# cloneofsimo/paint-with-words-sd

Hardware: NVIDIA H100
Metric: unet_steps_per_sec_512sq_cfg (higher is better)
Workload: dtype f16

## Files before the change

### paint_with_words_sd_b200/attention.py

```python
from __future__ import annotations

import math
from typing import Dict, Optional, Union

import torch
import torch.nn.functional as F

from . import _native
from .conditioning import PACK_TOKENS, expand_orig_weight_map, key_chunks, pack_weight_map, packed_key, weight_key
from .weight_function import g_of_sigma, probe_weight_function

_ORIG_KEY = "CROSS_ATTENTION_WEIGHT_ORIG"
RECORD_KEY = "ATTN_RECORD"


class _DeviceState:

    def __init__(self, device: torch.device):
        self.device = device
        self.g_sigma = torch.zeros(1, dtype=torch.float32, device=device)
        self._g_key = None
        self.stats = torch.zeros(1024, dtype=torch.float32, device=device)
        self.workspace = torch.zeros(8 << 20, dtype=torch.uint8, device=device)
        self.fused_ws = torch.zeros(_native.lib().pww_xattn_fused_workspace_bytes(), dtype=torch.uint8, device=device)
        self.index_cache: Dict[int, torch.Tensor] = {}
        self.pack_cache: Dict[tuple, object] = {}

    def set_g(self, key, value: float) -> None:
        if key != self._g_key:
            self.g_sigma.fill_(value)
            self._g_key = key

    def ensure(self, batch: int, ws_bytes: int) -> None:
        if self.stats.numel() < batch or self.workspace.numel() < ws_bytes:
            raise _native.NativeError(f"batch of {batch} images exceeds the shim's fixed scratch; split the call or pass "
                                      "your own stats_out/workspace")

    def packed(self, wmap: torch.Tensor):
        key = (wmap.data_ptr(), wmap._version, tuple(wmap.shape), tuple(wmap.stride()))
        hit = self.pack_cache.get(key)
        if hit is None:
            if torch.cuda.is_current_stream_capturing():
                raise _native.NativeError("weight map must be packed before CUDA-graph capture (run one eager step first "
                                          "or pass packed maps)")
            while len(self.pack_cache) >= 16:
                self.pack_cache.pop(next(iter(self.pack_cache)))
            hit = (wmap, pack_weight_map(wmap) or False)
            self.pack_cache[key] = hit
        return hit[1] or None

    def shared_index(self, batch: int) -> torch.Tensor:
        t = self.index_cache.get(batch)
        if t is None:
            t = torch.zeros(batch, dtype=torch.int32, device=self.device)
            self.index_cache[batch] = t
        return t


_STATES: Dict[torch.device, _DeviceState] = {}


def _state(device: torch.device) -> _DeviceState:
    s = _STATES.get(device)
    if s is None:
        s = _STATES[device] = _DeviceState(device)
    return s


def reset_device_state() -> None:
    _STATES.clear()


def resolve_weight_map(context: dict, n: int, device):
    try:
        return context[weight_key(n)]
    except KeyError:
        w = context[_ORIG_KEY]
        if isinstance(w, int):
            if context.get("ORIG_FALLBACK_DROPPED"):
                raise NotImplementedError(
                    f"no CROSS_ATTENTION_WEIGHT_{n} in a multi-image context: the ORIG-map fallback (paint_with_words.py:97-103) "
                    "is a single-image path; use sizes divisible by 64 or one image per sampler")
            return 0
        w = expand_orig_weight_map(w.detach().to("cpu", torch.float32), n).to(device)
        context[weight_key(n)] = w
        return w


def _elem_dtype(q: torch.Tensor) -> torch.dtype:
    return torch.bfloat16 if q.dtype == torch.bfloat16 else torch.float16


def _autocast_dtype(module) -> torch.dtype:
    return torch.bfloat16 if module.to_q.weight.dtype == torch.bfloat16 else torch.float16


def _rows(t: torch.Tensor, dtype: torch.dtype = torch.float16) -> torch.Tensor:
    if t.dtype != dtype:
        t = t.to(dtype)
    if t.stride(-1) != 1 or (t.stride(0) % 8) or (t.stride(1) % 8) or (t.data_ptr() % 16):
        t = t.contiguous()
    return t


XATTN_IMPL = "auto"


def cross_attention(q: torch.Tensor, k: torch.Tensor, v: torch.Tensor, heads: int, scale: float,
                    wmap: Optional[torch.Tensor] = None, wmap_index: Optional[torch.Tensor] = None,
                    stat: Union[int, torch.Tensor] = _native.PWW_STAT_MAX, g_sigma: Optional[torch.Tensor] = None,
                    return_stats: bool = False, packed=None, stats_out: Optional[torch.Tensor] = None,
                    workspace: Optional[torch.Tensor] = None, record=None):
    L = _native.lib()
    dt = _elem_dtype(q)
    q, k, v = _rows(q, dt), _rows(k, dt), _rows(v, dt)
    B, N, C = q.shape
    T = k.shape[1]
    D = C // heads
    if k.stride() != v.stride():
        v = v.contiguous()
        k = k.contiguous()
    st = _state(q.device)
    with torch.cuda.device(q.device):
        out = torch.empty((B, N, C), dtype=dt, device=q.device)
        stream = torch.cuda.current_stream(q.device).cuda_stream
        biased = wmap is not None or packed is not None
        if wmap is not None:
            if wmap.dim() == 2:
                wmap = wmap.unsqueeze(0)
            if wmap.shape[1] != N or wmap.shape[2] != T:
                raise ValueError(f"weight map shape {tuple(wmap.shape)} does not match N={N}, T={T}")
        impl = "dense" if XATTN_IMPL == "dense" else "fused"
        if impl == "dense" and biased and wmap is None:
            impl = "fused"
        if biased and packed is None and impl == "fused":
            if wmap.dtype != torch.float32 or not wmap.is_contiguous():
                wmap = wmap.to(torch.float32).contiguous()
            packed = st.packed(wmap)
        use_fused = impl == "fused" and (not biased or packed is not None)
        if biased and wmap_index is None:
            bw = packed[0].shape[0] if packed is not None else wmap.shape[0]
            wmap_index = st.shared_index(B) if bw == 1 else torch.arange(B, dtype=torch.int32, device=q.device)
        per_image = isinstance(stat, torch.Tensor)
        kind_ptr = None
        if per_image and biased:
            if (stat.dtype != torch.int32 or stat.numel() != B or not stat.is_contiguous() or stat.device != q.device
                    or g_sigma is None or g_sigma.dtype != torch.float32 or g_sigma.numel() != B
                    or not g_sigma.is_contiguous() or g_sigma.device != q.device):
                raise ValueError(f"per-image settings need an int32 [{B}] kind tensor and an fp32 [{B}] G tensor on "
                                 f"{q.device}")
            kind_ptr = stat.data_ptr()
        stats = None
        rec_args = ()
        if record is not None:
            if not use_fused:
                why = ("XATTN_IMPL is 'dense'" if impl == "dense" else
                       "the weight map has more than 10 distinct columns and takes the dense two-launch path")
                raise _native.NativeError(f"attention recording needs the one-launch kernel, but {why}")
            ridx, rec_index, rec_acc = record
            if (ridx.dtype != torch.int8 or ridx.dim() != 2 or ridx.shape[1] != PACK_TOKENS * max(1, key_chunks(T))
                    or not ridx.is_contiguous() or rec_index.dtype != torch.int32 or rec_index.numel() != B
                    or not rec_index.is_contiguous() or rec_acc.dtype != torch.float32 or rec_acc.dim() != 4
                    or tuple(rec_acc.shape[1:]) != (heads, N, 16) or not rec_acc[0].is_contiguous()
                    or any(t.device != q.device for t in (ridx, rec_index, rec_acc))):
                raise ValueError(f"record needs int8 [Br, {PACK_TOKENS * max(1, key_chunks(T))}] ridx, int32 [{B}] "
                                 f"rec_index and fp32 [Br, {heads}, {N}, 16] rec_acc on {q.device}")
            if not per_image and biased:
                stat = torch.full((B,), int(stat), dtype=torch.int32, device=q.device)
                g_sigma = g_sigma.reshape(-1)[:1].expand(B).contiguous()
                kind_ptr, per_image = stat.data_ptr(), True
            rec_args = (ridx.data_ptr(), rec_index.data_ptr(), rec_acc.data_ptr(), rec_acc.stride(0))
        if use_fused:
            mp_ptr = ci_ptr = idx_ptr = g_ptr = st_ptr = ws_ptr = None
            mp_bs = bw = ws_bytes = 0
            if biased:
                mpack, cidx = packed
                if (mpack.shape[1] != N or mpack.dtype != torch.float16 or cidx.dtype != torch.int8
                        or cidx.shape[-1] != PACK_TOKENS * max(1, key_chunks(T))):
                    raise ValueError("packed weight map does not match this attention level")
                st.ensure(B, 0)
                stats = st.stats if stats_out is None else stats_out
                ws = st.fused_ws if workspace is None else workspace
                mp_ptr, ci_ptr, idx_ptr = mpack.data_ptr(), cidx.data_ptr(), wmap_index.data_ptr()
                g_ptr, st_ptr, ws_ptr = g_sigma.data_ptr(), stats.data_ptr(), ws.data_ptr()
                mp_bs, bw, ws_bytes = mpack.stride(0), mpack.shape[0], ws.numel()
            name = "pww_xattn_fused_rec" if rec_args else ("pww_xattn_fused_multi" if per_image else "pww_xattn_fused")
            fn = _native.entry(name, dt)
            rc = fn(q.data_ptr(), k.data_ptr(), v.data_ptr(), out.data_ptr(), B, heads, N, T, D,
                    q.stride(0), q.stride(1), k.stride(0), k.stride(1), out.stride(0), out.stride(1),
                    mp_ptr, mp_bs, bw, ci_ptr, idx_ptr, kind_ptr if per_image or rec_args else stat, g_ptr,
                    float(scale), st_ptr, ws_ptr, ws_bytes, stream, *rec_args)
            _native.check(rc, fn.__name__)
            _native.launch_count += 1
        else:
            stats_ptr = g_ptr = w_ptr = idx_ptr = None
            w_bs = 0
            if biased:
                if wmap is None:
                    raise ValueError("the dense path needs the dense weight map")
                if wmap.dtype != torch.float32 or not wmap.is_contiguous():
                    wmap = wmap.to(torch.float32).contiguous()
                ws_bytes = L.pww_xattn_workspace_bytes(B, heads, N, T, D)
                st.ensure(B, ws_bytes)
                stats = st.stats if stats_out is None else stats_out
                fn = _native.entry("pww_xattn_stats_multi" if per_image else "pww_xattn_stats", dt)
                rc = fn(q.data_ptr(), k.data_ptr(), B, heads, N, T, D, q.stride(0), q.stride(1), k.stride(0),
                        k.stride(1), kind_ptr if per_image else stat, wmap_index.data_ptr(), stats.data_ptr(),
                        st.workspace.data_ptr(), st.workspace.numel(), stream)
                _native.check(rc, fn.__name__)
                _native.launch_count += 1
                stats_ptr, g_ptr = stats.data_ptr(), g_sigma.data_ptr()
                w_ptr, idx_ptr, w_bs = wmap.data_ptr(), wmap_index.data_ptr(), wmap.stride(0)
            fn = _native.entry("pww_xattn_fwd_multi" if per_image else "pww_xattn_fwd", dt)
            rc = fn(q.data_ptr(), k.data_ptr(), v.data_ptr(), out.data_ptr(), B, heads, N, T, D,
                    q.stride(0), q.stride(1), k.stride(0), k.stride(1), out.stride(0), out.stride(1),
                    w_ptr, w_bs, idx_ptr, stats_ptr, g_ptr, float(scale), stream)
            _native.check(rc, fn.__name__)
            _native.launch_count += 1
    if return_stats:
        return out, (stats[:B].clone() if stats is not None else None)
    return out


SELF_ATTN_IMPL = "auto"
SELF_ATTN_NATIVE_MAX_KEYS = 1024


def self_attention(q: torch.Tensor, k: torch.Tensor, v: torch.Tensor, heads: int, scale: float) -> torch.Tensor:
    B, N, C = q.shape
    D = C // heads
    if SELF_ATTN_IMPL == "native" or (SELF_ATTN_IMPL == "auto" and N <= SELF_ATTN_NATIVE_MAX_KEYS):
        dt = _elem_dtype(q)
        fn = _native.entry("pww_attn_fwd", dt)
        q, k, v = _rows(q, dt), _rows(k, dt), _rows(v, dt)
        if not (q.stride() == k.stride() == v.stride()):
            q, k, v = q.contiguous(), k.contiguous(), v.contiguous()
        with torch.cuda.device(q.device):
            out = torch.empty((B, N, C), dtype=dt, device=q.device)
            rc = fn(q.data_ptr(), k.data_ptr(), v.data_ptr(), out.data_ptr(), B, heads, N, D,
                    q.stride(0), q.stride(1), out.stride(0), out.stride(1), float(scale),
                    torch.cuda.current_stream(q.device).cuda_stream)
        _native.check(rc, fn.__name__)
        _native.launch_count += 1
        return out
    qh = q.reshape(B, N, heads, D).transpose(1, 2)
    kh = k.reshape(B, k.shape[1], heads, D).transpose(1, 2)
    vh = v.reshape(B, v.shape[1], heads, D).transpose(1, 2)
    o = F.scaled_dot_product_attention(qh, kh, vh, scale=scale)
    return o.transpose(1, 2).reshape(B, N, C)


def _fused_weight(module, attr: str, names) -> torch.Tensor:
    params = [getattr(module, n).weight for n in names]
    key = tuple((p.data_ptr(), p._version, p.dtype, p.device) for p in params)
    hit = getattr(module, attr, None)
    if hit is None or hit[0] != key:
        hit = (key, torch.cat(params, 0).detach().contiguous())
        object.__setattr__(module, attr, hit)
    return hit[1]


def refresh_kv_cache(context: dict) -> None:
    cache = context.get("KV_CACHE")
    if not cache:
        return
    ctx = context["CONTEXT_TENSOR"]
    for module, kv in cache.values():
        with torch.autocast("cuda", dtype=_autocast_dtype(module)):
            kv.copy_(F.linear(ctx, _fused_weight(module, "_pww_wkv", ("to_k", "to_v"))))


def inj_forward(self, hidden_states, context=None, mask=None):
    if not hidden_states.is_cuda:
        raise _native.NativeError("paint_with_words_sd_b200 attention runs on an H100 GPU only (no CPU path)")
    is_dict = isinstance(context, dict)
    if context is None:
        ctx = hidden_states
    else:
        ctx = context["CONTEXT_TENSOR"] if is_dict else context

    C = self.to_q.weight.shape[0]
    act = _autocast_dtype(self)
    with torch.autocast("cuda", dtype=act):
        if context is None:
            qkv = F.linear(hidden_states, _fused_weight(self, "_pww_wqkv", ("to_q", "to_k", "to_v")))
            q, k, v = qkv[..., :C], qkv[..., C:2 * C], qkv[..., 2 * C:]
        else:
            q = self.to_q(hidden_states)
            cache = context.get("KV_CACHE") if is_dict else None
            hit = cache.get(id(self)) if cache is not None else None
            if hit is not None:
                kv = hit[1]
            else:
                kv = F.linear(ctx, _fused_weight(self, "_pww_wkv", ("to_k", "to_v")))
                if cache is not None:
                    cache[id(self)] = (self, kv)
            k, v = kv[..., :C], kv[..., C:]

    if context is None:
        o = self_attention(q, k, v, self.heads, self.scale)
    else:
        wmap = wmap_index = g_dev = packed = None
        scratch = (None, None)
        stat = _native.PWW_STAT_MAX
        kinds = context.get("STAT_KIND") if is_dict else None
        if kinds is not None:
            w = resolve_weight_map(context, q.shape[1], q.device)
            if isinstance(w, torch.Tensor):
                wmap, stat, g_dev = w, kinds, context["G_SIGMA"]
                wmap_index = context.get("WMAP_INDEX")
                packed = context.get(packed_key(q.shape[1]))
                scratch = context.get("PWW_SCRATCH", scratch)
        elif is_dict:
            f = context["WEIGHT_FUNCTION"]
            sigma = context["SIGMA"]
            w = resolve_weight_map(context, q.shape[1], q.device)
            probed = probe_weight_function(f, sigma)
            if isinstance(w, torch.Tensor) and not probed.is_zero:
                g_dev = context.get("G_SIGMA")
                if g_dev is None:
                    st = _state(q.device)
                    st.set_g((id(f), float(sigma)), g_of_sigma(f, probed, sigma))
                    g_dev = st.g_sigma
                wmap, stat = w, probed.stat
                wmap_index = context.get("WMAP_INDEX")
                packed = context.get(packed_key(q.shape[1]))
                scratch = context.get("PWW_SCRATCH", scratch)
        record = None
        recs = context.get(RECORD_KEY) if is_dict else None
        if recs is not None:
            record = recs.get(q.shape[1])
            if record is None:
                raise _native.NativeError(f"attention recording has no accumulator for N = {q.shape[1]} query rows "
                                          f"(levels: {sorted(recs)})")
        if k.shape[0] != q.shape[0]:
            k = k.expand(q.shape[0], -1, -1)
            v = v.expand(q.shape[0], -1, -1)
        o = cross_attention(q, k, v, self.heads, self.scale, wmap, wmap_index, stat, g_dev, packed=packed,
                            stats_out=scratch[0], workspace=scratch[1], record=record)

    with torch.autocast("cuda", dtype=act):
        o = self.to_out[0](o)
        o = self.to_out[1](o)
    return o


class PwWAttnProcessor:

    def __call__(self, attn, hidden_states, encoder_hidden_states=None, attention_mask=None, **kwargs):
        return inj_forward(attn, hidden_states, encoder_hidden_states, attention_mask)


_PATCHED: Dict[type, object] = {}


def patch_unet(unet, forward=inj_forward) -> int:
    count = 0
    for m in unet.modules():
        if m.__class__.__name__ == "CrossAttention":
            cls = m.__class__
            if cls not in _PATCHED:
                _PATCHED[cls] = cls.__dict__.get("__call__")
            cls.__call__ = forward
            count += 1
    return count


def unpatch_all() -> None:
    for cls, orig in _PATCHED.items():
        if orig is None:
            if "__call__" in cls.__dict__:
                delattr(cls, "__call__")
        else:
            cls.__call__ = orig
    _PATCHED.clear()
```

### paint_with_words_sd_b200/csrc/attn_tc.cuh

```cuda
#pragma once
#include "mma_sm90.cuh"
#include "pww_common.cuh"
#include "xattn_core.cuh"

namespace pww {
namespace fa {

constexpr int kThreads = core::kThreads;
constexpr int kBM = core::kBM;
constexpr int kBN = 64;

template <int D>
struct Cfg {
  using T_ = core::Tile<D>;
  static constexpr uint32_t KVBYTES = kBN * T_::LD * 2;
  static constexpr uint32_t OFF_KV = T_::QBYTES;
  static constexpr uint32_t SMEM = T_::QBYTES + 2 * 2 * KVBYTES;
  static_assert(SMEM <= 232448, "shared memory budget");
};

template <typename E>
struct Params {
  const E* q;
  const E* k;
  const E* v;
  E* out;
  int B, H, N;
  int64_t bs, rs;
  int64_t o_bs, o_rs;
  float scale;
};

template <int D, typename E>
constexpr int kMinBlocks = (D == 80 && std::is_same_v<E, __nv_bfloat16>) ? 1 : 0;

template <int D, typename E>
__global__ void __launch_bounds__(kThreads, kMinBlocks<D, E>) attn_fwd_kernel(const Params<E> p) {
  using C = core::Tile<D>;
  using CF = Cfg<D>;
  extern __shared__ __align__(128) unsigned char smem[];
  const uint32_t smem0 = ptx::smem_u32(smem);
  const int warp = threadIdx.x >> 5, lane = threadIdx.x & 31;
  const int qtiles = (p.N + kBM - 1) / kBM;
  const int bh = blockIdx.x / qtiles, qt = blockIdx.x - bh * qtiles;
  const int b = bh / p.H, h = bh - b * p.H;
  const int row_base = qt * kBM;
  const E* qb = p.q + (int64_t)b * p.bs + h * D;
  const E* kb = p.k + (int64_t)b * p.bs + h * D;
  const E* vb = p.v + (int64_t)b * p.bs + h * D;
  const int ntiles = (p.N + kBN - 1) / kBN;
  auto issue_kv = [&](int j) {
    const uint32_t st = smem0 + CF::OFF_KV + (j & 1) * 2 * CF::KVBYTES;
    const int rows = p.N - j * kBN < kBN ? p.N - j * kBN : kBN;
    core::load_rows<D>(st, kb + (int64_t)j * kBN * p.rs, p.rs, kBN, rows);
    core::load_rows<D>(st + CF::KVBYTES, vb + (int64_t)j * kBN * p.rs, p.rs, kBN, rows);
    ptx::cp_async_commit();
  };
  {
    const int rows = p.N - row_base < kBM ? p.N - row_base : kBM;
    core::load_rows<D>(smem0, qb + (int64_t)row_base * p.rs, p.rs, kBM, rows);
  }
  issue_kv(0);
  uint32_t qa[C::KS][4];
  float o[C::NT][4], m0, m1, l0, l1;
  core::warp_online_begin<D>(o, m0, m1, l0, l1);
  const float sl2 = p.scale * 1.4426950408889634f;
  const uint32_t qs = smem0 + (uint32_t)(warp * 16 * C::LD) * 2u;
#pragma unroll 1
  for (int jt = 0; jt < ntiles; ++jt) {
    if (jt + 1 < ntiles) {
      issue_kv(jt + 1);
      ptx::cp_async_wait<1>();
    } else {
      ptx::cp_async_wait<0>();
    }
    __syncthreads();
    if (jt == 0) {
#pragma unroll
      for (int kk = 0; kk < C::KS; ++kk)
        ptx::ldsm_x4(qs + (uint32_t)((lane & 15) * C::LD + kk * 16 + (lane >> 4) * 8) * 2u, qa[kk][0], qa[kk][1], qa[kk][2], qa[kk][3]);
    }
    const uint32_t ks = smem0 + CF::OFF_KV + (jt & 1) * 2 * CF::KVBYTES, vs = ks + CF::KVBYTES;
    float s[kBN / 8][4];
#pragma unroll
    for (int j = 0; j < kBN / 8; ++j) s[j][0] = s[j][1] = s[j][2] = s[j][3] = 0.f;
#pragma unroll
    for (int kk = 0; kk < C::KS; ++kk) {
#pragma unroll
      for (int jp = 0; jp < kBN / 16; ++jp) {
        const int t = 16 * jp + (lane & 7) + ((lane >> 4) << 3), d = kk * 16 + ((lane >> 3) & 1) * 8;
        uint32_t b0, b1, b2, b3;
        ptx::ldsm_x4(ks + (uint32_t)(t * C::LD + d) * 2u, b0, b1, b2, b3);
        ptx::mma16816<E>(s[2 * jp], qa[kk], b0, b1);
        ptx::mma16816<E>(s[2 * jp + 1], qa[kk], b2, b3);
      }
    }
    core::warp_online_chunk<D, E>(s, p.N - jt * kBN, sl2, vs, lane, o, m0, m1, l0, l1);
    __syncthreads();
  }
  core::warp_online_end<D>(o, l0, l1);
  core::warp_store<D>(o, smem + warp * 16 * C::LD * 2, lane, p.out + (int64_t)b * p.o_bs + h * D, p.o_rs,
                      row_base + warp * 16, p.N);
}

template <int D, typename E>
cudaError_t launch(const void* q, const void* k, const void* v, void* out, int B, int H, int N, int64_t bs, int64_t rs,
                   int64_t o_bs, int64_t o_rs, float scale, cudaStream_t s) {
  using CF = Cfg<D>;
  Params<E> p;
  p.q = (const E*)q; p.k = (const E*)k; p.v = (const E*)v; p.out = (E*)out;
  p.B = B; p.H = H; p.N = N; p.bs = bs; p.rs = rs; p.o_bs = o_bs; p.o_rs = o_rs; p.scale = scale;
  const cudaError_t e = allow_dynamic_smem<attn_fwd_kernel<D, E>>(CF::SMEM);
  if (e != cudaSuccess) return e;
  const long long grid = (long long)B * H * ((N + kBM - 1) / kBM);
  if (grid > 0x7fffffffLL) return cudaErrorInvalidConfiguration;
  attn_fwd_kernel<D, E><<<(unsigned)grid, kThreads, CF::SMEM, s>>>(p);
  return cudaGetLastError();
}

}
}
```

Before: 160.2.

## Split keys across warps, add multistage KV pipeline and ones-column row sums

Rewrites the native self-attention kernel. For short sequences (N<=256) the warps are split into two groups over key blocks and their partial results are merged through shared memory. It adds a 3-stage cp.async pipeline where it fits, and computes the softmax denominator by padding V with a ones column, so the row sum falls out of the PV MMA. It also lowers the native self-attention threshold from 1024 to 256 keys, so the 512px levels with 1024 and 4096 tokens now take the fallback (likely SDPA) path. That trades a small extra MMA column and a combine step for more parallelism on small N.

```diff
diff --git a/paint_with_words_sd_b200/attention.py b/paint_with_words_sd_b200/attention.py
--- a/paint_with_words_sd_b200/attention.py
+++ b/paint_with_words_sd_b200/attention.py
@@ -223,7 +223,7 @@
 
 
 SELF_ATTN_IMPL = "auto"
-SELF_ATTN_NATIVE_MAX_KEYS = 1024
+SELF_ATTN_NATIVE_MAX_KEYS = 256
 
 
 def self_attention(q: torch.Tensor, k: torch.Tensor, v: torch.Tensor, heads: int, scale: float) -> torch.Tensor:
diff --git a/paint_with_words_sd_b200/csrc/attn_tc.cuh b/paint_with_words_sd_b200/csrc/attn_tc.cuh
--- a/paint_with_words_sd_b200/csrc/attn_tc.cuh
+++ b/paint_with_words_sd_b200/csrc/attn_tc.cuh
@@ -7,16 +7,26 @@
 namespace fa {
 
 constexpr int kThreads = core::kThreads;
-constexpr int kBM = core::kBM;
-constexpr int kBN = 64;
-
-template <int D>
+constexpr int kWarps = core::kWarps;
+constexpr uint32_t kSmemMax = 232448;
+
+template <int D, int S, int BN>
 struct Cfg {
+  static_assert(S == 1 || S == 2, "key splits");
+  static_assert(BN % 16 == 0, "P V takes 16 keys per k-step");
   using T_ = core::Tile<D>;
-  static constexpr uint32_t KVBYTES = kBN * T_::LD * 2;
-  static constexpr uint32_t OFF_KV = T_::QBYTES;
-  static constexpr uint32_t SMEM = T_::QBYTES + 2 * 2 * KVBYTES;
-  static_assert(SMEM <= 232448, "shared memory budget");
+  static constexpr int R = kWarps / S;
+  static constexpr int BM = 16 * R;
+  static constexpr int KB = S * BN;
+  static constexpr int NV = T_::NT + 1;
+  static constexpr uint32_t QBYTES = BM * T_::LD * 2;
+  static constexpr uint32_t KVBYTES = KB * T_::LD * 2;
+  static constexpr uint32_t OFF_KV = QBYTES;
+  static constexpr int STAGES = QBYTES + 3 * 2 * KVBYTES <= kSmemMax ? 3 : 2;
+  static constexpr uint32_t SMEM = QBYTES + STAGES * 2 * KVBYTES;
+  static constexpr int PART = NV * 4 + 2;
+  static_assert(SMEM <= kSmemMax, "shared memory budget");
+  static_assert(S == 1 || (uint32_t)(kWarps - R) * 32 * PART * 4 <= STAGES * 2 * KVBYTES, "combine buffer");
 };
 
 template <typename E>
@@ -34,89 +44,227 @@
 template <int D, typename E>
 constexpr int kMinBlocks = (D == 80 && std::is_same_v<E, __nv_bfloat16>) ? 1 : 0;
 
-template <int D, typename E>
+template <int D, int NROWS, typename E>
+__device__ __forceinline__ void load_kv(uint32_t dst, const E* src, int64_t rs, int valid) {
+  using C = core::Tile<D>;
+  constexpr int DCH = D / 8, PIECES = NROWS * DCH;
+#pragma unroll
+  for (int i = 0; i < (PIECES + kThreads - 1) / kThreads; ++i) {
+    const int idx = threadIdx.x + i * kThreads;
+    if (PIECES % kThreads != 0 && idx >= PIECES) break;
+    const int r = idx / DCH, c = idx - r * DCH;
+    const bool ok = r < valid;
+    ptx::cp_async16(dst + (uint32_t)(r * C::LD + c * 8) * 2u, ok ? (const void*)(src + (int64_t)r * rs + c * 8) : (const void*)src,
+                    ok ? 16u : 0u);
+  }
+}
+
+template <int D, typename E, int BN, int NV>
+__device__ __forceinline__ void warp_tile(const uint32_t (&qa)[core::Tile<D>::KS][4], uint32_t ks, uint32_t vs, int kv,
+                                          float sl2, int lane, float (&o)[NV][4], float& m0, float& m1) {
+  using C = core::Tile<D>;
+  constexpr int NJ = BN / 8;
+  float s[NJ][4];
+#pragma unroll
+  for (int j = 0; j < NJ; ++j) s[j][0] = s[j][1] = s[j][2] = s[j][3] = 0.f;
+#pragma unroll
+  for (int kk = 0; kk < C::KS; ++kk) {
+#pragma unroll
+    for (int jp = 0; jp < NJ / 2; ++jp) {
+      const int t = 16 * jp + (lane & 7) + ((lane >> 4) << 3), d = kk * 16 + ((lane >> 3) & 1) * 8;
+      uint32_t b0, b1, b2, b3;
+      ptx::ldsm_x4(ks + (uint32_t)(t * C::LD + d) * 2u, b0, b1, b2, b3);
+      ptx::mma16816<E>(s[2 * jp], qa[kk], b0, b1);
+      ptx::mma16816<E>(s[2 * jp + 1], qa[kk], b2, b3);
+    }
+  }
+  if (kv < BN) {
+#pragma unroll
+    for (int j = 0; j < NJ; ++j)
+#pragma unroll
+      for (int e = 0; e < 4; ++e)
+        if (core::tok(j, e, lane) >= kv) s[j][e] = -INFINITY;
+  }
+  float t0 = -INFINITY, t1 = -INFINITY;
+#pragma unroll
+  for (int j = 0; j < NJ; ++j) {
+    t0 = fmaxf(t0, fmaxf(s[j][0], s[j][1]));
+    t1 = fmaxf(t1, fmaxf(s[j][2], s[j][3]));
+  }
+  t0 = fmaxf(t0, __shfl_xor_sync(0xffffffffu, t0, 1));
+  t0 = fmaxf(t0, __shfl_xor_sync(0xffffffffu, t0, 2));
+  t1 = fmaxf(t1, __shfl_xor_sync(0xffffffffu, t1, 1));
+  t1 = fmaxf(t1, __shfl_xor_sync(0xffffffffu, t1, 2));
+  const float mn0 = fmaxf(m0, t0), mn1 = fmaxf(m1, t1);
+  if (__any_sync(0xffffffffu, mn0 != m0 || mn1 != m1)) {
+    const float a0 = ptx::ex2((m0 - mn0) * sl2), a1 = ptx::ex2((m1 - mn1) * sl2);
+#pragma unroll
+    for (int j = 0; j < NV; ++j) {
+      o[j][0] *= a0; o[j][1] *= a0; o[j][2] *= a1; o[j][3] *= a1;
+    }
+  }
+  m0 = mn0; m1 = mn1;
+  const float n0 = -mn0 * sl2, n1 = -mn1 * sl2;
+  uint32_t pa[NJ / 2][4];
+#pragma unroll
+  for (int j = 0; j < NJ; ++j) {
+    pa[j >> 1][(j & 1) * 2] = ptx::pack2<E>(ptx::ex2(fmaf(s[j][0], sl2, n0)), ptx::ex2(fmaf(s[j][1], sl2, n0)));
+    pa[j >> 1][(j & 1) * 2 + 1] = ptx::pack2<E>(ptx::ex2(fmaf(s[j][2], sl2, n1)), ptx::ex2(fmaf(s[j][3], sl2, n1)));
+  }
+#pragma unroll
+  for (int kk = 0; kk < NJ / 2; ++kk) {
+    const int t = 16 * kk + (lane & 7) + ((lane >> 3) & 1) * 8;
+#pragma unroll
+    for (int jp = 0; jp < NV / 2; ++jp) {
+      uint32_t b0, b1, b2, b3;
+      ptx::ldsm_x4_t(vs + (uint32_t)(t * C::LD + 16 * jp + (lane >> 4) * 8) * 2u, b0, b1, b2, b3);
+      ptx::mma16816<E>(o[2 * jp], pa[kk], b0, b1);
+      ptx::mma16816<E>(o[2 * jp + 1], pa[kk], b2, b3);
+    }
+    if constexpr (NV & 1) {
+      uint32_t b0, b1;
+      ptx::ldsm_x2_t(vs + (uint32_t)(t * C::LD + 8 * (NV - 1)) * 2u, b0, b1);
+      ptx::mma16816<E>(o[NV - 1], pa[kk], b0, b1);
+    }
+  }
+}
+
+template <int D, typename E, int S, int BN>
 __global__ void __launch_bounds__(kThreads, kMinBlocks<D, E>) attn_fwd_kernel(const Params<E> p) {
   using C = core::Tile<D>;
-  using CF = Cfg<D>;
+  using CF = Cfg<D, S, BN>;
+  constexpr int NV = CF::NV, STAGES = CF::STAGES;
   extern __shared__ __align__(128) unsigned char smem[];
   const uint32_t smem0 = ptx::smem_u32(smem);
   const int warp = threadIdx.x >> 5, lane = threadIdx.x & 31;
-  const int qtiles = (p.N + kBM - 1) / kBM;
+  const int split = warp / CF::R, slice = warp - split * CF::R;
+  const int qtiles = (p.N + CF::BM - 1) / CF::BM;
   const int bh = blockIdx.x / qtiles, qt = blockIdx.x - bh * qtiles;
   const int b = bh / p.H, h = bh - b * p.H;
-  const int row_base = qt * kBM;
+  const int row_base = qt * CF::BM;
   const E* qb = p.q + (int64_t)b * p.bs + h * D;
   const E* kb = p.k + (int64_t)b * p.bs + h * D;
   const E* vb = p.v + (int64_t)b * p.bs + h * D;
-  const int ntiles = (p.N + kBN - 1) / kBN;
-  auto issue_kv = [&](int j) {
-    const uint32_t st = smem0 + CF::OFF_KV + (j & 1) * 2 * CF::KVBYTES;
-    const int rows = p.N - j * kBN < kBN ? p.N - j * kBN : kBN;
-    core::load_rows<D>(st, kb + (int64_t)j * kBN * p.rs, p.rs, kBN, rows);
-    core::load_rows<D>(st + CF::KVBYTES, vb + (int64_t)j * kBN * p.rs, p.rs, kBN, rows);
-    ptx::cp_async_commit();
+  const int nstages = (p.N + CF::KB - 1) / CF::KB;
+  for (int r = threadIdx.x; r < STAGES * 2 * CF::KB; r += kThreads) {
+    const int slot = r / (2 * CF::KB), i = r - slot * 2 * CF::KB;
+    const uint4 pad = make_uint4(i >= CF::KB ? ptx::pack2<E>(1.f, 0.f) : 0u, 0u, 0u, 0u);
+    *reinterpret_cast<uint4*>(smem + CF::OFF_KV + slot * 2 * CF::KVBYTES + (i * C::LD + D) * 2) = pad;
+  }
+  auto issue_kv = [&](int i) {
+    const uint32_t st = smem0 + CF::OFF_KV + (i % STAGES) * 2 * CF::KVBYTES;
+    const int rows = p.N - i * CF::KB;
+    load_kv<D, CF::KB>(st, kb + (int64_t)i * CF::KB * p.rs, p.rs, rows);
+    load_kv<D, CF::KB>(st + CF::KVBYTES, vb + (int64_t)i * CF::KB * p.rs, p.rs, rows);
   };
   {
-    const int rows = p.N - row_base < kBM ? p.N - row_base : kBM;
-    core::load_rows<D>(smem0, qb + (int64_t)row_base * p.rs, p.rs, kBM, rows);
+    const int rows = p.N - row_base < CF::BM ? p.N - row_base : CF::BM;
+    core::load_rows<D>(smem0, qb + (int64_t)row_base * p.rs, p.rs, CF::BM, rows);
   }
   issue_kv(0);
+  ptx::cp_async_commit();
+#pragma unroll
+  for (int i = 1; i < STAGES - 1; ++i) {
+    if (i < nstages) issue_kv(i);
+    ptx::cp_async_commit();
+  }
   uint32_t qa[C::KS][4];
-  float o[C::NT][4], m0, m1, l0, l1;
-  core::warp_online_begin<D>(o, m0, m1, l0, l1);
+  float o[NV][4], m0 = -INFINITY, m1 = -INFINITY;
+#pragma unroll
+  for (int j = 0; j < NV; ++j) o[j][0] = o[j][1] = o[j][2] = o[j][3] = 0.f;
   const float sl2 = p.scale * 1.4426950408889634f;
-  const uint32_t qs = smem0 + (uint32_t)(warp * 16 * C::LD) * 2u;
+  const uint32_t qs = smem0 + (uint32_t)(slice * 16 * C::LD) * 2u;
 #pragma unroll 1
-  for (int jt = 0; jt < ntiles; ++jt) {
-    if (jt + 1 < ntiles) {
-      issue_kv(jt + 1);
-      ptx::cp_async_wait<1>();
-    } else {
-      ptx::cp_async_wait<0>();
-    }
+  for (int it = 0; it < nstages; ++it) {
+    ptx::cp_async_wait<STAGES - 2>();
     __syncthreads();
-    if (jt == 0) {
+    if (it == 0) {
 #pragma unroll
       for (int kk = 0; kk < C::KS; ++kk)
         ptx::ldsm_x4(qs + (uint32_t)((lane & 15) * C::LD + kk * 16 + (lane >> 4) * 8) * 2u, qa[kk][0], qa[kk][1], qa[kk][2], qa[kk][3]);
     }
-    const uint32_t ks = smem0 + CF::OFF_KV + (jt & 1) * 2 * CF::KVBYTES, vs = ks + CF::KVBYTES;
-    float s[kBN / 8][4];
-#pragma unroll
-    for (int j = 0; j < kBN / 8; ++j) s[j][0] = s[j][1] = s[j][2] = s[j][3] = 0.f;
-#pragma unroll
-    for (int kk = 0; kk < C::KS; ++kk) {
-#pragma unroll
-      for (int jp = 0; jp < kBN / 16; ++jp) {
-        const int t = 16 * jp + (lane & 7) + ((lane >> 4) << 3), d = kk * 16 + ((lane >> 3) & 1) * 8;
-        uint32_t b0, b1, b2, b3;
-        ptx::ldsm_x4(ks + (uint32_t)(t * C::LD + d) * 2u, b0, b1, b2, b3);
-        ptx::mma16816<E>(s[2 * jp], qa[kk], b0, b1);
-        ptx::mma16816<E>(s[2 * jp + 1], qa[kk], b2, b3);
+    if (it + STAGES - 1 < nstages) issue_kv(it + STAGES - 1);
+    ptx::cp_async_commit();
+    const int kv = p.N - it * CF::KB - split * BN;
+    if (kv > 0) {
+      const uint32_t ks = smem0 + CF::OFF_KV + (it % STAGES) * 2 * CF::KVBYTES + (uint32_t)(split * BN * C::LD) * 2u;
+      warp_tile<D, E, BN, NV>(qa, ks, ks + CF::KVBYTES, kv, sl2, lane, o, m0, m1);
+    }
+  }
+  if constexpr (S > 1) {
+    ptx::cp_async_wait<0>();
+    __syncthreads();
+    float* part = reinterpret_cast<float*>(smem + CF::OFF_KV);
+    if (split > 0) {
+      float* w = part + ((split - 1) * CF::R + slice) * 32 * CF::PART + lane;
+#pragma unroll
+      for (int j = 0; j < NV; ++j)
+#pragma unroll
+        for (int e = 0; e < 4; ++e) w[(4 * j + e) * 32] = o[j][e];
+      w[4 * NV * 32] = m0;
+      w[(4 * NV + 1) * 32] = m1;
+    }
+    __syncthreads();
+    if (split > 0) return;
+    float mt0 = m0, mt1 = m1;
+#pragma unroll
+    for (int sp = 1; sp < S; ++sp) {
+      const float* w = part + ((sp - 1) * CF::R + slice) * 32 * CF::PART + lane;
+      mt0 = fmaxf(mt0, w[4 * NV * 32]);
+      mt1 = fmaxf(mt1, w[(4 * NV + 1) * 32]);
+    }
+    {
+      const float a0 = ptx::ex2((m0 - mt0) * sl2), a1 = ptx::ex2((m1 - mt1) * sl2);
+#pragma unroll
+      for (int j = 0; j < NV; ++j) {
+        o[j][0] *= a0; o[j][1] *= a0; o[j][2] *= a1; o[j][3] *= a1;
       }
     }
-    core::warp_online_chunk<D, E>(s, p.N - jt * kBN, sl2, vs, lane, o, m0, m1, l0, l1);
-    __syncthreads();
-  }
-  core::warp_online_end<D>(o, l0, l1);
-  core::warp_store<D>(o, smem + warp * 16 * C::LD * 2, lane, p.out + (int64_t)b * p.o_bs + h * D, p.o_rs,
-                      row_base + warp * 16, p.N);
-}
+#pragma unroll
+    for (int sp = 1; sp < S; ++sp) {
+      const float* w = part + ((sp - 1) * CF::R + slice) * 32 * CF::PART + lane;
+      const float a0 = ptx::ex2((w[4 * NV * 32] - mt0) * sl2), a1 = ptx::ex2((w[(4 * NV + 1) * 32] - mt1) * sl2);
+#pragma unroll
+      for (int j = 0; j < NV; ++j) {
+        o[j][0] = fmaf(w[(4 * j) * 32], a0, o[j][0]);
+        o[j][1] = fmaf(w[(4 * j + 1) * 32], a0, o[j][1]);
+        o[j][2] = fmaf(w[(4 * j + 2) * 32], a1, o[j][2]);
+        o[j][3] = fmaf(w[(4 * j + 3) * 32], a1, o[j][3]);
+      }
+    }
+  }
+  const float i0 = 1.f / __shfl_sync(0xffffffffu, o[NV - 1][0], lane & ~3);
+  const float i1 = 1.f / __shfl_sync(0xffffffffu, o[NV - 1][2], lane & ~3);
+  float on[C::NT][4];
+#pragma unroll
+  for (int j = 0; j < C::NT; ++j) {
+    on[j][0] = o[j][0] * i0; on[j][1] = o[j][1] * i0; on[j][2] = o[j][2] * i1; on[j][3] = o[j][3] * i1;
+  }
+  core::warp_store<D>(on, smem + slice * 16 * C::LD * 2, lane, p.out + (int64_t)b * p.o_bs + h * D, p.o_rs,
+                      row_base + slice * 16, p.N);
+}
+
+template <int D, typename E, int S, int BN>
+cudaError_t launch_cfg(const Params<E>& p, cudaStream_t s) {
+  using CF = Cfg<D, S, BN>;
+  const cudaError_t e = allow_dynamic_smem<attn_fwd_kernel<D, E, S, BN>>(CF::SMEM);
+  if (e != cudaSuccess) return e;
+  const long long grid = (long long)p.B * p.H * ((p.N + CF::BM - 1) / CF::BM);
+  if (grid > 0x7fffffffLL) return cudaErrorInvalidConfiguration;
+  attn_fwd_kernel<D, E, S, BN><<<(unsigned)grid, kThreads, CF::SMEM, s>>>(p);
+  return cudaGetLastError();
+}
+
+inline int splits_for(int N) { return N <= 256 ? 2 : 1; }
 
 template <int D, typename E>
 cudaError_t launch(const void* q, const void* k, const void* v, void* out, int B, int H, int N, int64_t bs, int64_t rs,
                    int64_t o_bs, int64_t o_rs, float scale, cudaStream_t s) {
-  using CF = Cfg<D>;
   Params<E> p;
   p.q = (const E*)q; p.k = (const E*)k; p.v = (const E*)v; p.out = (E*)out;
   p.B = B; p.H = H; p.N = N; p.bs = bs; p.rs = rs; p.o_bs = o_bs; p.o_rs = o_rs; p.scale = scale;
-  const cudaError_t e = allow_dynamic_smem<attn_fwd_kernel<D, E>>(CF::SMEM);
-  if (e != cudaSuccess) return e;
-  const long long grid = (long long)B * H * ((N + kBM - 1) / kBM);
-  if (grid > 0x7fffffffLL) return cudaErrorInvalidConfiguration;
-  attn_fwd_kernel<D, E><<<(unsigned)grid, kThreads, CF::SMEM, s>>>(p);
-  return cudaGetLastError();
-}
-
-}
-}
+  return splits_for(N) == 2 ? launch_cfg<D, E, 2, 64>(p, s) : launch_cfg<D, E, 1, 64>(p, s);
+}
+
+}
+}
```

Result: faster. 162.0, median of 6 (+1.1%).
